# wangheda/youtube-8m

Hardware: AMD Instinct MI355X
Metric: training videos/sec (higher is better)
Workload: dtype f32; 1 GPU; BASELINE configs[3]: LstmModel (2 x BasicLSTMCell(1024), dynamic_rnn over F=300) on raw uint8 [B,300,1152] frames + MoeModel head (2 mixtures, V=4716), fp32 training step (fwd+bwd+clip+Adam); per_gpu_batch=128, global_batch=128, frames=300, parallelism=dp1, params=113902808

## Files before the change

### include/yt8m_hip.h

```cpp
#ifndef YT8M_HIP_H
#define YT8M_HIP_H
#include <stdint.h>

#ifdef __cplusplus
extern "C" {
#endif

typedef void* yt8m_stream_t;

enum yt8m_status { YT8M_OK = 0, YT8M_E_BADARG = -1, YT8M_E_SHAPE = -2, YT8M_E_HIP = -3, YT8M_E_RCCL = -4 };
enum yt8m_label_dtype { YT8M_LABEL_U8 = 0, YT8M_LABEL_F32 = 1 };

int yt8m_abi_version(void);
const char* yt8m_last_error(void);
const char* yt8m_built_arch(void);

int yt8m_prof_enable(int on);
int yt8m_prof_reset(void);
int yt8m_prof_get(int family, int64_t* launches, double* total_ms);
int yt8m_prof_get_flops(int family, double* flops);
int yt8m_prof_get_bytes(int family, double* bytes);

int yt8m_probe_mfma_f32(int iters, int blocks, float* sink, yt8m_stream_t stream);
int yt8m_probe_mfma_bf16(int iters, int blocks, int random_operands, float* sink, yt8m_stream_t stream);
// ... 49 lines not shown
                          yt8m_stream_t stream);
int yt8m_timepool_shiftmax_f32(const float* z, int64_t F, int64_t B, int64_t ldz, int nfilt, const int32_t* fs, const int32_t* ncol, float* out,
                               int32_t* idx, int64_t ldo, yt8m_stream_t stream);
int yt8m_u8_cnn_pool_dw(const uint8_t* q, const float* r_tm, const int32_t* idx, const float* g, int64_t ldg, int64_t B, int64_t F, int64_t D,
                        int64_t N, int64_t fs, float* dW, float beta, yt8m_stream_t stream);
int yt8m_f32_cnn_pool_dw(const float* x, int64_t ldx, const int32_t* idx, const float* g, int64_t ldg, int64_t B, int64_t F, int64_t D,
                         int64_t N, int64_t fs, float* dW, int64_t lddw, float beta, yt8m_stream_t stream);
int yt8m_f32_cnn_pool_dx(const int32_t* idx, const float* g, int64_t ldg, int64_t B, int64_t F, int64_t D, int nfilt, const float* const* wt,
                         const int32_t* fs, const int32_t* ncol, float* dx, int64_t lddx, yt8m_stream_t stream);
int yt8m_u8_frames_image_f16(const uint8_t* q, const int32_t* num_frames, int64_t B, int64_t F, int64_t D, float eps, void* image,
                             float* x_tm, float* r_out, yt8m_stream_t stream);
int yt8m_u8_frames_image_t_f16(const uint8_t* q, const int32_t* num_frames, int64_t B, int64_t F, int64_t D, void* image_t,
                               yt8m_stream_t stream);
int yt8m_gemm_h2_nt_grouped(int nprob, const yt8m_gemm_problem* probs, const float* alphas, const float* const* dsa,
                            const float* const* dsb, void* workspace, int64_t workspace_bytes, yt8m_stream_t stream);
int yt8m_x3_set_combine(int mode);
int yt8m_x3_set_schedule(int mode);
#define YT8M_GEMM_ROLE_DW 0x100
#define YT8M_GEMM_ROLE_H2 0x200
int yt8m_gemm_x3_pays(int64_t M, int64_t N, int64_t K);
int64_t yt8m_gemm_auto_scratch_bytes(int transA, int transB, int nprob, const yt8m_gemm_problem* probs);
int yt8m_gemm_auto_grouped(int transA, int transB, int nprob, const yt8m_gemm_problem* probs, void* workspace,
                           int64_t workspace_bytes, void* image_scratch, int64_t image_scratch_bytes, uint64_t* used_x3,
                           yt8m_stream_t stream);
int yt8m_gemm_auto_grouped_ex(int transA, int transB, int nprob, const yt8m_gemm_problem* probs, const float* const* absmaxA,
                              const float* const* absmaxB, void* workspace, int64_t workspace_bytes, void* image_scratch,
                              int64_t image_scratch_bytes, uint64_t* used_x3, yt8m_stream_t stream);
int yt8m_gemm_x1x3_nt(int64_t M, int64_t N, int64_t K, const void* A1, const void* B3, float* C, int64_t ldc, const float* bias,
                      const float* rowscale, const float* colsum, float colsum_scale, void* workspace, int64_t workspace_bytes,
                      yt8m_stream_t stream);
// ... 332 lines not shown
int64_t yt8m_lstm_stack_tape_bytes(const yt8m_lstm_stack_desc* desc);
int64_t yt8m_lstm_stack_scratch_bytes(const yt8m_lstm_stack_desc* desc);
int yt8m_lstm_stack_partition(const yt8m_lstm_stack_desc* desc, int* fwd_chunks, int* bwd_chunks);
int yt8m_lstm_stack_streams(int L, yt8m_stream_t* layer_streams, yt8m_stream_t* wgrad_stream);
int yt8m_lstm_stack_fwd(const yt8m_lstm_stack_desc* desc, const void* x, const int32_t* num_frames, const float* const* W,
                        const float* const* b, void* tape, int64_t tape_bytes, void* scratch, int64_t scratch_bytes,
                        yt8m_stream_t stream);
int yt8m_lstm_stack_view(const yt8m_lstm_stack_desc* desc, void* tape, int layer, int which, float** out);
int yt8m_lstm_stack_bwd(const yt8m_lstm_stack_desc* desc, const void* x, const int32_t* num_frames, const float* const* W, void* tape,
                        int64_t tape_bytes, void* scratch, int64_t scratch_bytes, const float* dout_top,
                        const float* const* dc_final, const float* const* dh_final, float* const* dW, float* const* db,
                        const float* beta_W, const float* beta_b, float* dx, yt8m_stream_t stream);
int yt8m_lstm_stack_status(const yt8m_lstm_stack_desc* desc, void* scratch, yt8m_stream_t stream);
int yt8m_lstm_stack_layer_done_wait(int layer, yt8m_stream_t stream);
int yt8m_lstm_stack_use_streams(int set, int* previous);
typedef void (*yt8m_stream_hook)(void* user, yt8m_stream_t stream);
int yt8m_lstm_stack_set_prep_hook(yt8m_stream_hook hook, void* user);
typedef struct yt8m_opt_ranges {
  float* w;
  float* m;
  float* v;
  const float* g;
  const int32_t* chunks;
  const int32_t* tensor_chunk_start;
  const int32_t* tensor_chunk_start_host;
  const float* l2;
  float* partial;
  float* norms;
  const uint8_t* skip_tensor;
  const yt8m_wimg_job* jobs;
// ... 217 lines not shown
```

### youtube-8m_amd/_lib.py

```python
import ctypes
import os

_HERE = os.path.dirname(os.path.abspath(__file__))
LIB_PATH = os.environ.get("YT8M_LIB", os.path.join(_HERE, "libyt8m_hip.so"))

c_void_p, c_int, c_int64, c_float, c_double = ctypes.c_void_p, ctypes.c_int, ctypes.c_int64, ctypes.c_float, ctypes.c_double
P = c_void_p

class GemmProblem(ctypes.Structure):
    _fields_ = [("M", c_int64), ("N", c_int64), ("K", c_int64), ("A", c_void_p), ("lda", c_int64), ("B", c_void_p),
                ("ldb", c_int64), ("C", c_void_p), ("ldc", c_int64), ("bias", c_void_p), ("beta", c_float)]


STREAM_HOOK = ctypes.CFUNCTYPE(None, ctypes.c_void_p, ctypes.c_void_p)


class PersistBwdImages(ctypes.Structure):
    _fields_ = [("plain", ctypes.c_void_p), ("trans", ctypes.c_void_p), ("trans_scaled", ctypes.c_void_p), ("rowscale", ctypes.c_void_p),
                ("colpart", ctypes.c_void_p), ("colpart_scaled", ctypes.c_void_p)]


class LstmStackDesc(ctypes.Structure):
    _fields_ = [("B", c_int64), ("F", c_int64), ("D", c_int64), ("H", c_int64), ("L", ctypes.c_int32), ("input_u8", ctypes.c_int32),
                ("forget_bias", c_float), ("fwd_chunks", ctypes.c_int32), ("bwd_chunks", ctypes.c_int32), ("need_dx", ctypes.c_int32),
# ... 283 lines not shown
    "yt8m_gemm_h1x2_nt_ex": (c_int, [c_int64, c_int64, c_int64, P, c_int64, P, c_int64, P, c_int64, P, c_float, P, P, P, c_float, c_float, P,
                                     c_int64, P]),
    "yt8m_h2_rowscales": (c_int, [P, c_int64, c_int64, c_int64, P, P, P]),
    "yt8m_h2_split_rows": (c_int, [P, c_int64, c_int64, c_int64, P, P, P]),
    "yt8m_gemm_h2_nt_ex": (c_int, [c_int64, c_int64, c_int64, P, c_int64, P, c_int64, P, c_int64, P, c_float, P, P, P, c_float, P, c_int64, P]),
    "yt8m_timepool_max_f32": (c_int, [P, c_int64, c_int64, c_int64, c_int64, P, P, c_int64, P]),
    "yt8m_timepool_shiftmax_f32": (c_int, [P, c_int64, c_int64, c_int64, c_int, ctypes.POINTER(ctypes.c_int32), ctypes.POINTER(ctypes.c_int32), P, P,
                                           c_int64, P]),
    "yt8m_u8_cnn_pool_dw": (c_int, [P, P, P, P, c_int64, c_int64, c_int64, c_int64, c_int64, c_int64, P, c_float, P]),
    "yt8m_f32_cnn_pool_dw": (c_int, [P, c_int64, P, P, c_int64, c_int64, c_int64, c_int64, c_int64, c_int64, P, c_int64, c_float, P]),
    "yt8m_f32_cnn_pool_dx": (c_int, [P, P, c_int64, c_int64, c_int64, c_int64, c_int, PP, ctypes.POINTER(ctypes.c_int32),
                                     ctypes.POINTER(ctypes.c_int32), P, c_int64, P]),
    "yt8m_u8_frames_image_f16": (c_int, [P, P, c_int64, c_int64, c_int64, c_float, P, P, P, P]),
    "yt8m_u8_frames_image_t_f16": (c_int, [P, P, c_int64, c_int64, c_int64, P, P]),
    "yt8m_gemm_h2_nt_grouped": (c_int, [c_int, ctypes.POINTER(GemmProblem), ctypes.POINTER(c_float), PP, PP, P, c_int64, P]),
    "yt8m_topk_rows": (c_int, [P, c_int64, c_int64, c_int, P, P, P]),
    "yt8m_perr_rows": (c_int, [P, P, c_int64, c_int64, P, P]),
    "yt8m_reverse_sequence_u8": (c_int, [P, P, P, c_int64, c_int64, c_int64, P]),
    "yt8m_reverse_sequence_f32_tm": (c_int, [P, c_int64, P, P, c_int64, c_int64, c_int64, c_int64, c_int64, P]),
    "yt8m_lstm_stack_use_streams": (c_int, [c_int, ctypes.POINTER(c_int)]),
    "yt8m_half_segments_u8": (c_int, [P, P, P, P, c_int64, c_int64, c_int64, P]),
    "yt8m_half_segments_f32": (c_int, [P, P, P, P, c_int64, c_int64, c_int64, P]),
    "yt8m_half_segment_means_u8": (c_int, [P, P, P, c_int64, c_int64, c_int64, c_int, c_float, P]),
    "yt8m_dequant_noise_u8": (c_int, [P, P, P, c_int64, c_int64, c_int64, c_float, ctypes.c_uint64, P]),
    "yt8m_resolution_mean_u8": (c_int, [P, P, P, P, c_int64, c_int64, c_int64, c_int64, c_int, c_float, P]),
    "yt8m_resolution_mean_f32": (c_int, [P, P, P, P, c_int64, c_int64, c_int64, c_int64, c_int, c_float, P]),
    "yt8m_multiscale_workspace_bytes": (c_int64, [c_int64]),
    "yt8m_colmoments_f32": (c_int, [P, c_int64, c_int64, c_int64, P, P, c_int, c_float, c_float, P, P, P, c_int64, P]),
    "yt8m_bn_relu_pool2_tm_fwd": (c_int, [P, c_int64, c_int64, c_int64, c_int64, P, P, P, P, P, c_int64, P, c_int64, P]),
    "yt8m_bn_relu_pool2_tm_bwd": (c_int, [P, c_int64, c_int64, c_int64, c_int64, P, P, P, P, c_int, P, c_int64, P, c_int64, P, c_int64, P,
# ... 73 lines not shown
```

### youtube-8m_amd/csrc/gemm_x3.hip

```cpp
#include "common.h"
#include "x3_image.h"
#include "philox.h"
#include <type_traits>
#include <algorithm>
#include <mutex>
#include <stdlib.h>

namespace {

constexpr int TM = 256, TN = 256;
constexpr int PLANE_F = 256 * 8;
constexpr int OP_F = 3 * PLANE_F;
constexpr int NST = 3;
using yt8m_x3::RG_F;
using yt8m_x3::store_block;

typedef float f32x16 __attribute__((ext_vector_type(16)));
typedef __bf16 bf16x8 __attribute__((ext_vector_type(8)));

struct XArgs {
  const float* A;
  const float* B;
  float* C;
  const float* bias;
  int64_t ldc;
  int M, N, KB;
  int ska, skb;
  int tiles_m, tiles_n;
  int accumulate;
  const float* rscale;
  const float* cs;
  float cs_scale;
  float alpha;
  const float* dsa;
  const float* dsb;
  int c_bf16;
};
__device__ __forceinline__ unsigned c_bf16_bits(float f) {
  unsigned u = __float_as_uint(f);
  if ((u & 0x7fffffffu) > 0x7f800000u) return (u >> 16) | 0x40u;
  u += 0x7fffu + ((u >> 16) & 1u);
  return u >> 16;
}
__device__ __forceinline__ void store_c4(const XArgs& g, int64_t off, float4 v) {
  if (g.c_bf16) {
    uint2 w;
    w.x = c_bf16_bits(v.x) | (c_bf16_bits(v.y) << 16);
    w.y = c_bf16_bits(v.z) | (c_bf16_bits(v.w) << 16);
    *reinterpret_cast<uint2*>(reinterpret_cast<unsigned short*>(g.C) + off) = w;
  } else {
    *reinterpret_cast<float4*>(g.C + off) = v;
// ... 513 lines not shown
      step(kt + 1, a0y, b2y, a0x, b2x, variant);
    }
    if (kt < nk) step(kt, a0x, b2x, a0y, b2y, variant);
  };
  if (grp == 0) run(std::integral_constant<int, 0>{});
  else run(std::integral_constant<int, 1>{});
  asm volatile("s_waitcnt lgkmcnt(0)" ::: "memory");
  __builtin_amdgcn_s_barrier();

  x_epilogue(G, g, acc, smem, m0, n0, wm, wn, lane, wave, li, lk, nparts, slot, q, lt);
}

typedef _Float16 f16x8 __attribute__((ext_vector_type(8)));

template <int PA>
__global__ __launch_bounds__(512) void gemm_h2q_kernel(const XGroup G) {
  constexpr int OPA_F = PA * PLANE_F;
  constexpr int H2_STAGE_F = (PA + 2) * PLANE_F;
  extern __shared__ __attribute__((aligned(16))) float smem[];
  int q, nparts, part, slot, lt;
  x_work_item(G, q, nparts, part, slot, lt);
  const XArgs& g = G.p[q];
  int tm, tn;
  tile_coords(g.tiles_m, g.tiles_n, lt, tm, tn);
  const int m0 = tm * TM, n0 = tn * TN;
  const int tid = threadIdx.x, lane = tid & 63, wave = tid >> 6;
  const int grp = wave >> 2;
  const int wm = grp * 128, wn = (wave & 3) * 64;
  const int li = lane & 31, lk = lane >> 5;
  const int kb0 = (int)((int64_t)g.KB * part / nparts), kb1 = (int)((int64_t)g.KB * (part + 1) / nparts);
  const int nk = kb1 - kb0;
  const float* pa = g.A + (int64_t)min(m0 / 32 + wave, (g.M + 31) / 32 - 1) * g.ska * (PA * RG_F) + lane * 4;
  const float* pb = g.B + (int64_t)min(n0 / 32 + wave, (g.N + 31) / 32 - 1) * g.skb * (2 * RG_F) + lane * 4;
  constexpr int DMA = PA + 2;
  f32x16 acc[4][2];
#pragma unroll
// ... 99 lines not shown
    int kt = 0;
    for (; kt + 1 < nk; kt += 2) {
      step(kt, ahx, blx, ahy, bly, variant);
      step(kt + 1, ahy, bly, ahx, blx, variant);
    }
    if (kt < nk) step(kt, ahx, blx, ahy, bly, variant);
  };
  if (grp == 0) run(std::integral_constant<int, 0>{});
  else run(std::integral_constant<int, 1>{});
  asm volatile("s_waitcnt lgkmcnt(0)" ::: "memory");
  __builtin_amdgcn_s_barrier();

  const XArgs ge = fold_device_scales(g);
  x_epilogue(G, ge, acc, smem, m0, n0, wm, wn, lane, wave, li, lk, nparts, slot, q, lt);
}

constexpr int B1_KBS = 4;
constexpr int B1_STAGE_F = 2 * B1_KBS * PLANE_F;

__global__ __launch_bounds__(512) void gemm_b1_kernel(const XGroup G) {
  extern __shared__ __attribute__((aligned(16))) float smem[];
  int q, nparts, part, slot, lt;
  x_work_item(G, q, nparts, part, slot, lt);
  const XArgs& g = G.p[q];
  int tm, tn;
  tile_coords(g.tiles_m, g.tiles_n, lt, tm, tn);
  const int m0 = tm * TM, n0 = tn * TN;
  const int tid = threadIdx.x, lane = tid & 63, wave = tid >> 6;
  const int wm = (wave >> 2) * 128, wn = (wave & 3) * 64;
  const int li = lane & 31, lk = lane >> 5;
// ... 627 lines not shown
        return nullptr;
      }
      base[dev] = p;
    }
    if (next[dev] + (uint32_t)n > CNT_CAP) next[dev] = 0;
    unsigned* r = base[dev] + next[dev];
    next[dev] += (uint32_t)n;
    return r;
  }
};
TileCounters g_cnt;

template <int PA>
int x3_launch(int nprob, const yt8m_gemm_problem* probs, const float* rscale, const float* cs, float cs_scale, float alpha,
              void* workspace, int64_t workspace_bytes, yt8m_stream_t stream, const float* const* dsa = nullptr,
              const float* const* dsb = nullptr, const float* alphas = nullptr, unsigned c_bf16_mask = 0) {
  XGroup G;
  G.nprob = 0;
  static const int SLOTS_ENV = getenv("YT8M_X3_SLOTS") ? atoi(getenv("YT8M_X3_SLOTS")) : 0;
  const int SLOTS = SLOTS_ENV >= 32 && SLOTS_ENV <= 256 ? SLOTS_ENV : 256;
  const int64_t per_part = (int64_t)TM * TN * sizeof(float);
  int64_t nfull = 0, slots = 0, fix = 0;
  for (int i = 0; i < nprob; ++i) {
    const yt8m_gemm_problem& q = probs[i];
    YT8M_REQUIRE(q.M >= 0 && q.N >= 0 && q.K >= 1 && q.ldc >= q.N, YT8M_E_BADARG, "bad GEMM problem");
    YT8M_REQUIRE(q.beta == 0.f || q.beta == 1.f, YT8M_E_BADARG, "beta must be 0 or 1");
    if (q.M == 0 || q.N == 0) continue;
    YT8M_REQUIRE(q.A && q.B && q.C, YT8M_E_BADARG, "null operand");
    YT8M_REQUIRE((((uintptr_t)q.A | (uintptr_t)q.B) & 15) == 0, YT8M_E_BADARG, "x3 images must be 16-byte aligned");
    XArgs g;
    g.A = static_cast<const float*>(q.A); g.B = static_cast<const float*>(q.B); g.C = q.C; g.bias = q.bias;
    g.ldc = q.ldc;
    g.M = (int)q.M; g.N = (int)q.N; g.KB = (int)((q.K + 15) / 16);
    YT8M_REQUIRE(q.lda >= 0 && q.ldb >= 0 && q.lda < (1LL << 30) && q.ldb < (1LL << 30) && (q.lda == 0 || q.lda >= g.KB) &&
                 (q.ldb == 0 || q.ldb >= g.KB), YT8M_E_BADARG, "bad image K-block stride");
    YT8M_REQUIRE((q.lda <= g.KB && q.ldb <= g.KB) || (q.K % 16) == 0, YT8M_E_SHAPE, "a K range of a larger image must be a multiple of 16");
    g.ska = q.lda ? (int)q.lda : g.KB; g.skb = q.ldb ? (int)q.ldb : g.KB;
    g.tiles_m = (int)((q.M + TM - 1) / TM); g.tiles_n = (int)((q.N + TN - 1) / TN);
    g.accumulate = q.beta != 0.f;
    g.rscale = rscale; g.cs = cs; g.cs_scale = cs_scale; g.alpha = alphas ? alphas[i] : alpha;
    g.dsa = dsa ? dsa[i] : nullptr; g.dsb = dsb ? dsb[i] : nullptr;
    g.c_bf16 = (int)((c_bf16_mask >> i) & 1u);
    YT8M_REQUIRE(!g.c_bf16 || (q.beta == 0.f && (q.ldc & 3) == 0 && ((uintptr_t)q.C & 15) == 0), YT8M_E_BADARG,
                 "a bf16 output takes beta = 0, ldc % 4 == 0 and a 16-byte aligned C");
    YT8M_REQUIRE(!(g.dsa || g.dsb || g.alpha != 1.0f) || (q.N % 4) == 0, YT8M_E_SHAPE, "a scaled product needs N % 4 == 0");
    const int64_t T = (int64_t)g.tiles_m * g.tiles_n;
    const int full = (int)(T / SLOTS) * SLOTS, rem = (int)(T - full);
    int S = 1;
    if (workspace && rem > 0) {
      double best = 1e30;
      for (int c = 1; c <= 16; ++c) {
        if (c > 1 && (g.KB / c < (PA == 0 ? 32 : 8) || (slots + (int64_t)rem * c) * per_part > workspace_bytes)) break;
        const int rounds = (rem * c + SLOTS - 1) / SLOTS;
        const double cost = rounds * ((double)g.KB / c + 10.0) + (c > 1 ? 4.0 + 0.065 * rem * c : 0.0);
        if (cost < best * 0.98) { best = cost; S = c; }
      }
    }
// ... 6 lines not shown
    G.part_base[k] = (int)slots;
    G.slot_base[k] = (int)slots;
    G.fix_base[k] = (int)fix;
    nfull += G.full[k];
    if (S > 1) { slots += (int64_t)rem * S; fix += rem; }
    ++G.nprob;
  }
  if (G.nprob == 0) return YT8M_OK;
  YT8M_REQUIRE(nfull + slots < (1LL << 30), YT8M_E_SHAPE, "too many tiles for one launch");
  for (int i = G.nprob; i <= 4; ++i) { G.full_base[i] = (int)nfull; G.part_base[i] = (int)slots; G.fix_base[i] = (int)fix; }
  for (int i = G.nprob; i < 4; ++i) { G.p[i] = G.p[0]; G.S[i] = 1; G.slot_base[i] = 0; G.full[i] = 0; G.rem[i] = 0; }
  G.ws = static_cast<float*>(workspace);
  G.cnt = fix > 0 ? g_cnt.take((int)fix) : nullptr;
  const int64_t grid = nfull + slots;
  constexpr int LDS_BYTES = PA == 0 ? 2 * B1_STAGE_F * (int)sizeof(float)
                            : PA == 2 ? NST * 4 * PLANE_F * (int)sizeof(float)
                            : PA == 4 ? NST * 3 * PLANE_F * (int)sizeof(float) : NST * (PA + 3) * PLANE_F * (int)sizeof(float);
  static DeviceOnce lds_once;
  if constexpr (PA == 0) YT8M_HIP_CHECK(lds_once.lds(reinterpret_cast<const void*>(gemm_b1_kernel), LDS_BYTES));
  else if constexpr (PA == 2) YT8M_HIP_CHECK(lds_once.lds(reinterpret_cast<const void*>(gemm_h2q_kernel<2>), LDS_BYTES));
  else if constexpr (PA == 4) YT8M_HIP_CHECK(lds_once.lds(reinterpret_cast<const void*>(gemm_h2q_kernel<1>), LDS_BYTES));
  else YT8M_HIP_CHECK(lds_once.lds(reinterpret_cast<const void*>(gemm_x3_kernel<(PA == 1) ? 1 : 3>), LDS_BYTES));
  double fl = 0.0;
  for (int i = 0; i < nprob; ++i) fl += 2.0 * (double)probs[i].M * (double)probs[i].N * (double)probs[i].K;
  ProfScope prof(PA == 0 ? F_GEMM : (PA == 1 ? F_GEMM_X1X3 : (PA == 2 ? F_GEMM_H2 : (PA == 4 ? F_GEMM_H1X2 : F_GEMM_X3))), as_stream(stream), fl);
  static const bool piped_env = getenv("YT8M_B1_PIPE") == nullptr || atoi(getenv("YT8M_B1_PIPE")) != 0;
  const bool piped = g_schedule_mode == 1 || (g_schedule_mode == 0 && piped_env);
  const char* launched = "gemm_x3_kernel";
  if constexpr (PA == 0) {
    launched = piped ? "gemm_b1q_kernel" : "gemm_b1_kernel";
    if (piped) {
      static DeviceOnce lds_once_q;
      YT8M_HIP_CHECK(lds_once_q.lds(reinterpret_cast<const void*>(gemm_b1q_kernel), BQ_SLOTS * BQ_SLOT_F * (int)sizeof(float)));
      hipLaunchKernelGGL(gemm_b1q_kernel, dim3((unsigned)grid), dim3(512), BQ_SLOTS * BQ_SLOT_F * (int)sizeof(float), as_stream(stream), G);
    } else {
      hipLaunchKernelGGL(gemm_b1_kernel, dim3((unsigned)grid), dim3(512), LDS_BYTES, as_stream(stream), G);
    }
  }
  else if constexpr (PA == 2) {
    launched = "gemm_h2q_kernel";
    hipLaunchKernelGGL(gemm_h2q_kernel<2>, dim3((unsigned)grid), dim3(512), LDS_BYTES, as_stream(stream), G);
  }
  else if constexpr (PA == 4) {
    launched = "gemm_h2q_kernel";
    hipLaunchKernelGGL(gemm_h2q_kernel<1>, dim3((unsigned)grid), dim3(512), LDS_BYTES, as_stream(stream), G);
  }
  else {
    static const bool xpiped_env = getenv("YT8M_X3_PIPE") == nullptr || atoi(getenv("YT8M_X3_PIPE")) != 0;
    const bool xpiped = g_schedule_mode == 1 || (g_schedule_mode == 0 && xpiped_env);
    launched = xpiped ? "gemm_x3q_kernel" : "gemm_x3_kernel";
    if (xpiped) {
      static DeviceOnce lds_once_xq;
      YT8M_HIP_CHECK(lds_once_xq.lds(reinterpret_cast<const void*>(gemm_x3q_kernel<(PA == 1) ? 1 : 3>), LDS_BYTES));
      hipLaunchKernelGGL(gemm_x3q_kernel<(PA == 1) ? 1 : 3>, dim3((unsigned)grid), dim3(512), LDS_BYTES, as_stream(stream), G);
    } else {
      hipLaunchKernelGGL(gemm_x3_kernel<(PA == 1) ? 1 : 3>, dim3((unsigned)grid), dim3(512), LDS_BYTES, as_stream(stream), G);
    }
  }
  if (fix > 0 && !G.cnt) hipLaunchKernelGGL(x3_fixup_kernel, dim3((unsigned)fix * 16), dim3(256), 0, as_stream(stream), G);
  return launch_status(launched);
}
// ... 23 lines not shown
  return x3_launch<0>(nprob, probs, nullptr, nullptr, 0.f, 1.0f, workspace, workspace_bytes, stream);
}

extern "C" int yt8m_gemm_b1_nt_grouped_bf16c(int nprob, const yt8m_gemm_problem* probs, unsigned c_bf16_mask, void* workspace,
                                             int64_t workspace_bytes, yt8m_stream_t stream) {
  YT8M_REQUIRE(nprob >= 1 && nprob <= 4 && probs, YT8M_E_BADARG, "1..4 problems per launch");
  return x3_launch<0>(nprob, probs, nullptr, nullptr, 0.f, 1.0f, workspace, workspace_bytes, stream, nullptr, nullptr, nullptr, c_bf16_mask);
}

extern "C" int yt8m_gemm_h2_nt_grouped(int nprob, const yt8m_gemm_problem* probs, const float* alphas, const float* const* dsa,
                                       const float* const* dsb, void* workspace, int64_t workspace_bytes, yt8m_stream_t stream) {
  YT8M_REQUIRE(nprob >= 1 && nprob <= 4 && probs, YT8M_E_BADARG, "1..4 problems per launch");
  return x3_launch<2>(nprob, probs, nullptr, nullptr, 0.f, 1.0f, workspace, workspace_bytes, stream, dsa, dsb, alphas);
}

extern "C" int yt8m_gemm_h2_nt_ex(int64_t M, int64_t N, int64_t K, const void* A2, int64_t ska, const void* B2, int64_t skb, float* C,
                                  int64_t ldc, const float* bias, float alpha, const void* dsa, const void* dsb, const float* rowscale,
                                  float beta, void* workspace, int64_t workspace_bytes, yt8m_stream_t stream) {
  YT8M_REQUIRE((N % 4) == 0, YT8M_E_SHAPE, "the scaled epilogue needs N % 4 == 0");
  yt8m_gemm_problem p;
  p.M = M; p.N = N; p.K = K; p.A = A2; p.lda = ska; p.B = B2; p.ldb = skb; p.C = C; p.ldc = ldc; p.bias = bias; p.beta = beta;
  const float* wa = static_cast<const float*>(dsa);
  const float* wb = static_cast<const float*>(dsb);
  return x3_launch<2>(1, &p, rowscale, nullptr, 0.f, alpha, workspace, workspace_bytes, stream, dsa ? &wa : nullptr, dsb ? &wb : nullptr);
}

extern "C" int yt8m_gemm_h1x2_nt_ex(int64_t M, int64_t N, int64_t K, const void* A1, int64_t ska, const void* B2, int64_t skb, float* C,
                                    int64_t ldc, const float* bias, float alpha, const void* dsb, const float* rowscale, const float* colsum,
                                    float colsum_scale, float beta, void* workspace, int64_t workspace_bytes, yt8m_stream_t stream) {
  YT8M_REQUIRE((N % 4) == 0, YT8M_E_SHAPE, "the scaled epilogue needs N % 4 == 0");
// ... 38 lines not shown
```

### youtube-8m_amd/csrc/lstm_stack.hip

```cpp
#include <stdlib.h>
#include <algorithm>
#include <mutex>
#include <vector>
#include "common.h"

using namespace yt8m;

namespace {

constexpr int MAXL = 8, MAXP = 64;
constexpr int MAXBP = 62;
constexpr float U8_ALPHA = 4.0f / 255.0f;
constexpr float U8_BETA = 128.0f * (4.0f / 255.0f) + (4.0f / 512.0f - 2.0f);
constexpr int64_t X3_MIN_ROWS = 1024;
constexpr int64_t STEP_IMAGES_MAX_BYTES = 8LL << 30;
constexpr float H2_S = 8192.0f;

int64_t up256(int64_t v) { return (v + 255) / 256 * 256; }

int knob(const char* name, int dflt) { const char* v = getenv(name); return v ? atoi(v) : dflt; }

struct Part { int64_t t0, T; };
int chunks(int64_t F, int n, Part* out) {
  if (n < 1) n = 1;
// ... 111 lines not shown
  int64_t fmax = 0, bmax = 0;
  for (int c = 0; c < p.nf; ++c) fmax = std::max(fmax, p.fp[c].T * p.B);
  for (int c = 0; c < p.nb; ++c) bmax = std::max(bmax, p.bp[c].T * p.B);
  for (int l = 0; l < p.L; ++l) {
    const int64_t Din = l ? p.H : p.D;
    const bool x1 = l == 0 && p.u8;
    p.wxt3[l] = o; o += x1 ? 0 : up256(ib(H4, Din));
    p.xi[l] = o; o += x1 ? 0 : up256(ib(fmax, Din));
    p.dz[l] = o; o += up256(FBH * 4 * 4);
    p.dbuf[l] = o; o += l + 1 < p.L ? up256(FBH * 4) : 0;
    p.work[l] = o; o += up256(4 * BH * 4);
    const bool dxl = l > 0 || p.need_dx;
    p.dz3[l] = o; o += dxl ? up256(ib(bmax, H4)) : 0;
    p.wx3[l] = o; o += dxl ? up256(ib(Din, H4)) : 0;
    p.xT[l] = o; o += x1 ? up256(x1_bytes(p.D, p.FB)) : up256(ib(Din, p.FB));
    p.hT[l] = o; o += up256(ib(p.H, p.FB));
  }
  p.h2 = (knob("YT8M_STACK_H2", 1) && !p.bf16) ? 1 : 0;
  p.keep = (d->input_keep_prob > 0.f && d->input_keep_prob < 1.f) ? d->input_keep_prob : 0.f;
  for (int l = 0; l < MAXL; ++l) p.seed[l] = d->dropout_seed[l];
  if (d->input_keep_prob < 0.f || d->input_keep_prob > 1.f) return "input_keep_prob must be in [0, 1]";
  if (p.keep > 0.f && (p.u8 || !p.h2 || p.keep < 0.3f || (p.D % 4) != 0 || (p.H % 4) != 0))
    return "input dropout: float input, f16 product forms (YT8M_STACK_H2), keep_prob >= 0.3, D % 4 == 0";
  p.img_rows = (knob("YT8M_STACK_FUSED_IMAGES", 0) && !p.bf16 && !p.h2) ? yt8m_lstm_persist_bwd_images_rows(p.B, p.H) : 0;
  const int64_t trows = p.img_rows ? p.FB : bmax;
  for (int l = 0; l < p.L; ++l) { p.dzT3[l] = o; o += up256(ib(H4, trows)); }
  p.dzT3s = o; o += p.u8 ? up256(ib(H4, trows)) : 0;
  const int64_t ci = p.img_rows ? up256((int64_t)p.img_rows * MAXP * 2 * H4 * 4) : 0;
  for (int l = 0; l < p.L; ++l) { p.cimg[l] = o; o += ci; }
  p.cimgs = o; o += p.u8 ? ci : 0;
  p.csr = o; o += up256(H4 * 4);
// ... 121 lines not shown

extern "C" int yt8m_lstm_stack_streams(int L, yt8m_stream_t* layer_streams, yt8m_stream_t* wgrad_stream) {
  YT8M_REQUIRE(L >= 1 && L <= MAXL && layer_streams, YT8M_E_BADARG, "1..8 layers, non-null output");
  std::lock_guard<std::mutex> lk(g_mu);
  DevState* S = nullptr;
  RC(dev_state(L, &S));
  for (int l = 0; l < L; ++l) layer_streams[l] = (yt8m_stream_t)S->rs[l];
  if (wgrad_stream) *wgrad_stream = (yt8m_stream_t)S->sw;
  return YT8M_OK;
}

extern "C" int yt8m_lstm_stack_use_streams(int set, int* previous) {
  YT8M_REQUIRE(set >= 0 && set < NSETS, YT8M_E_BADARG, "stream set must be 0 or 1");
  if (previous) *previous = g_set;
  g_set = set;
  return YT8M_OK;
}

extern "C" int yt8m_lstm_stack_view(const yt8m_lstm_stack_desc* desc, void* tape, int layer, int which, float** out) {
  Plan P;
  const char* why = plan(desc, &P);
  YT8M_REQUIRE(!why, YT8M_E_SHAPE, why ? why : "");
  YT8M_REQUIRE(tape && out && layer >= 0 && layer < P.L && which >= 0 && which <= 3, YT8M_E_BADARG, "bad view");
  const int64_t FBH = P.FB * P.H;
  switch (which) {
    case 0: *out = at<float>(tape, P.out[layer]); break;
    case 1: *out = at<float>(tape, P.cs[layer]) + FBH; break;
    case 2: *out = at<float>(tape, P.hs[layer]) + FBH; break;
    default: *out = at<float>(tape, P.z[layer]); break;
  }
// ... 218 lines not shown
  YT8M_REQUIRE(!P.need_dx || dx, YT8M_E_BADARG, "need_dx is set but dx is NULL");
  for (int l = 0; l < P.L; ++l) {
    YT8M_REQUIRE(W[l], YT8M_E_BADARG, "null weights");
    YT8M_REQUIRE(!beta_W || beta_W[l] == 0.f || beta_W[l] == 1.f, YT8M_E_BADARG, "beta must be 0 or 1");
    YT8M_REQUIRE(!beta_b || beta_b[l] == 0.f || beta_b[l] == 1.f, YT8M_E_BADARG, "beta must be 0 or 1");
  }
  std::lock_guard<std::mutex> lk(g_mu);
  DevState* S = nullptr;
  RC(dev_state(P.L, &S));
  Ev ev(*S, 1);
  hipStream_t main = as_stream(stream), sw = S->sw;
  static const int dx_stream = knob("YT8M_STACK_DX_STREAM", 0), two_sw = knob("YT8M_STACK_SW2", 0);
  const int fuse_dz = P.h2 ? 0 : knob("YT8M_STACK_FUSE_DZ_SPLIT", 0);
  const int64_t B = P.B, D = P.D, H = P.H, H4 = 4 * H, BH = B * H, FB = P.FB;
  const int64_t KBtot = FB / 16;
  const bool bf = P.bf16 != 0;
  const int64_t KBB = bf ? 1024 : 3072;
  auto split = [&](const float* src, int64_t R, int64_t C, int64_t ld, float scale, void* plain, void* trans, hipStream_t st) {
    return bf ? yt8m_bf16_image(src, R, C, ld, scale, plain, trans, (yt8m_stream_t)st) : yt8m_x3_split(src, R, C, ld, scale, plain, trans, (yt8m_stream_t)st);
  };
  auto gemm = [&](int n, const yt8m_gemm_problem* pr, void* ws, int64_t wsb, hipStream_t st) {
    return bf ? yt8m_gemm_b1_nt_grouped(n, pr, ws, wsb, (yt8m_stream_t)st) : yt8m_gemm_x3_nt_grouped(n, pr, ws, wsb, (yt8m_stream_t)st);
  };
  hipEvent_t start = ev.record(main);
  ev.wait(sw, start);
  if (two_sw) ev.wait(S->sw2, start);
  for (int l = 0; l < P.L; ++l) { ev.wait(S->rs[l], start); if (dx_stream) ev.wait(S->dxs[l], start); }
  if (P.h2)
    for (int l = 0; l < P.L; ++l) {
      YT8M_HIP_CHECK(hipMemsetAsync(at<char>(scratch, P.hsc + 256 * l + 4), 0, 248, S->rs[l]));
      if (P.emit_max && l >= 1) YT8M_HIP_CHECK(hipMemsetAsync(at<char>(scratch, P.rmax + l * P.rmax_stride), 0, (size_t)FB * 4, S->rs[l]));
    }
  for (int l = 0; l < P.L; ++l) {
    if (!dW[l]) continue;
    if (l == 0 && P.u8) {
      if (P.h2) RC(yt8m_u8_frames_image_t_f16(static_cast<const uint8_t*>(x), num_frames, B, P.F, D, at<char>(scratch, P.xT[0]), sw));
      else RC(yt8m_u8_frames_image_t(static_cast<const uint8_t*>(x), num_frames, B, P.F, D, at<char>(scratch, P.xT[0]), sw));
    } else {
      const float* src = l ? at<float>(tape, P.out[l - 1]) : static_cast<const float*>(x);
      const int64_t Din = l ? H : D;
      if (P.h2 && P.keep > 0.f)
        RC(yt8m_h2_split_dropout(src, FB, Din, l ? H2_S : 1.0f, l ? nullptr : at<float>(scratch, P.hx0), nullptr, at<char>(scratch, P.xT[l]),
                                 P.keep, P.seed[l], 0, (yt8m_stream_t)sw));
      else if (P.h2 && l >= 1) RC(yt8m_h2_split(src, FB, Din, Din, H2_S, nullptr, nullptr, at<char>(scratch, P.xT[l]), nullptr, (yt8m_stream_t)sw));
      else if (P.h2) RC(yt8m_h2_split(src, FB, Din, Din, 1.0f, at<float>(scratch, P.hx0), nullptr, at<char>(scratch, P.xT[0]), nullptr, (yt8m_stream_t)sw));
      else RC(split(src, FB, Din, Din, 1.0f, nullptr, at<char>(scratch, P.xT[l]), sw));
    }
    if (P.h2) RC(yt8m_h2_split(at<float>(tape, P.hs[l]), FB, H, H, H2_S, nullptr, nullptr, at<char>(scratch, P.hT[l]), nullptr, (yt8m_stream_t)sw));
    else RC(split(at<float>(tape, P.hs[l]), FB, H, H, 1.0f, nullptr, at<char>(scratch, P.hT[l]), sw));
  }
  yt8m_stream_hook hook = g_prep_hook;
  void* hook_user = g_prep_user;
  g_prep_hook = nullptr;
  g_prep_user = nullptr;
  bool early = g_early.set;
  g_early.set = false;
  if (two_sw) ev.wait(S->sw2, ev.record(sw));
  int phase[MAXL];
  bool wx3_done[MAXL];
  const void* wx_img[MAXL] = {nullptr};
  hipEvent_t dzT_free[MAXL] = {nullptr};
  const bool fused_img = P.img_rows > 0 && !dx_stream && !fuse_dz;
  int64_t img_done_rows[MAXL] = {0};
// ... 145 lines not shown
      }
      hipStream_t sw = (two_sw && l == 0) ? S->sw2 : S->sw;
      ev.wait(sw, rb);
      void* gw = at<char>(scratch, (two_sw && l == 0) ? P.gws2 : P.gws[P.L]);
      const float bW = first ? (beta_W ? beta_W[l] : 0.f) : 1.f;
      const bool lastpart = c == 0 && j == 0;
      if (dW[l]) {
        if (l == 0 && P.u8 && P.h2) {
          const float* rr = at<float>(tape, P.rrow) + t0 * B;
          float* word = at<float>(scratch, P.hsc) + 1 + c;
          if (!P.emit_max) RC(yt8m_h2_absmax(dzc, M, H4, H4, word, (yt8m_stream_t)sw));
          float* cp = P.colparts ? at<float>(scratch, P.cpart[l]) + (t0 * B / 64) * H4 : nullptr;
          float* cps = P.colparts ? at<float>(scratch, P.cparts) + (t0 * B / 64) * H4 : nullptr;
          RC(yt8m_h2_split_ex(dzc, M, H4, H4, 1.0f, word, rr, nullptr, at<char>(scratch, P.dzT3[l]), at<char>(scratch, P.dzT3s), cp, cps,
                              (yt8m_stream_t)sw));
          RC(yt8m_gemm_h1x2_nt_ex(D, H4, M, at<char>(scratch, P.xT[0]) + kb0 * 1024, KBtot, at<char>(scratch, P.dzT3s), 0, dW[0], H4, nullptr,
                                  U8_ALPHA, word, nullptr, nullptr, 0.f, bW, gw, P.gws_bytes, (yt8m_stream_t)sw));
          yt8m_gemm_problem pr = {H, H4, M, at<char>(scratch, P.hT[0]) + kb0 * 2048, KBtot, at<char>(scratch, P.dzT3[l]), 0,
                                  dW[0] + D * H4, H4, nullptr, bW};
          const float alpha = 1.0f / H2_S;
          const float* dsb = word;
          RC(yt8m_gemm_h2_nt_grouped(1, &pr, &alpha, nullptr, &dsb, gw, P.gws_bytes, (yt8m_stream_t)sw));
        } else if (l == 0 && P.u8) {
          const float* rr = at<float>(tape, P.rrow) + t0 * B;
          if (fused_img) {
          } else if (P.colparts || bf) {
            float* cp = P.colparts ? at<float>(scratch, P.cpart[l]) + (t0 * B / 64) * H4 : nullptr;
            float* cps = P.colparts ? at<float>(scratch, P.cparts) + (t0 * B / 64) * H4 : nullptr;
            if (bf) RC(yt8m_bf16_image_colsum(dzc, M, H4, H4, 1.0f, rr, nullptr, at<char>(scratch, P.dzT3[l]), at<char>(scratch, P.dzT3s), cp, cps, sw));
            else RC(yt8m_x3_split_colsum(dzc, M, H4, H4, 1.0f, rr, nullptr, at<char>(scratch, P.dzT3[l]), at<char>(scratch, P.dzT3s), cp, cps, sw));
          } else
            RC(yt8m_x3_split_ex(dzc, M, H4, H4, 1.0f, rr, nullptr, at<char>(scratch, P.dzT3[l]), at<char>(scratch, P.dzT3s), sw));
          if (bf)
            RC(yt8m_gemm_b1_nt_ex(D, H4, M, at<char>(scratch, P.xT[0]) + kb0 * 1024, KBtot, dzTs_img, 0, dW[0], H4,
                                  nullptr, U8_ALPHA, nullptr, nullptr, 0.f, bW, gw, P.gws_bytes, sw));
          else
            RC(yt8m_gemm_x1x3_nt_ex(D, H4, M, at<char>(scratch, P.xT[0]) + kb0 * 1024, KBtot, dzTs_img, 0, dW[0], H4,
                                    nullptr, U8_ALPHA, nullptr, nullptr, 0.f, bW, gw, P.gws_bytes, sw));
          yt8m_gemm_problem pr = {H, H4, M, at<char>(scratch, P.hT[0]) + kb0 * KBB, KBtot, dzT_img, 0,
                                  dW[0] + D * H4, H4, nullptr, bW};
          RC(gemm(1, &pr, gw, P.gws_bytes, sw));
        } else if (P.h2) {
          float* word = at<float>(scratch, P.hsc + 256 * l) + 1 + c;
          if (!P.emit_max) RC(yt8m_h2_absmax(dzc, M, H4, H4, word, (yt8m_stream_t)sw));
          float* cp = (P.colparts && db[l]) ? at<float>(scratch, P.cpart[l]) + (t0 * B / 64) * H4 : nullptr;
          RC(yt8m_h2_split(dzc, M, H4, H4, 1.0f, word, nullptr, at<char>(scratch, P.dzT3[l]), cp, (yt8m_stream_t)sw));
          yt8m_gemm_problem pr[2] = {
              {Din, H4, M, at<char>(scratch, P.xT[l]) + kb0 * 2048, KBtot, at<char>(scratch, P.dzT3[l]), 0, dW[l], H4, nullptr, bW},
              {H, H4, M, at<char>(scratch, P.hT[l]) + kb0 * 2048, KBtot, at<char>(scratch, P.dzT3[l]), 0, dW[l] + Din * H4, H4, nullptr, bW}};
          const float alphas[2] = {l ? 1.0f / H2_S : 1.0f, 1.0f / H2_S};
          const float* dsa[2] = {l ? nullptr : at<float>(scratch, P.hx0), nullptr};
          const float* dsb[2] = {word, word};
          RC(yt8m_gemm_h2_nt_grouped(2, pr, alphas, dsa, dsb, gw, P.gws_bytes, (yt8m_stream_t)sw));
        } else {
          if (fused_img) {
          } else if (!fused_t) {
            if (P.colparts && db[l]) {
              float* cp = at<float>(scratch, P.cpart[l]) + (t0 * B / 64) * H4;
              if (bf) RC(yt8m_bf16_image_colsum(dzc, M, H4, H4, 1.0f, nullptr, nullptr, at<char>(scratch, P.dzT3[l]), nullptr, cp, nullptr, sw));
              else RC(yt8m_x3_split_colsum(dzc, M, H4, H4, 1.0f, nullptr, nullptr, at<char>(scratch, P.dzT3[l]), nullptr, cp, nullptr, sw));
            } else {
              RC(split(dzc, M, H4, H4, 1.0f, nullptr, at<char>(scratch, P.dzT3[l]), sw));
            }
          }
// ... 42 lines not shown
```

Before: 8408 videos/s.

## Group layer-0 u8 dW GEMMs into one mixed-plane launch and share h-transpose images

Adds a mixed-plane grouped h2 GEMM kernel that dispatches per problem between 1-plane and 2-plane A operands, so the layer-0 input-weight and recurrent-weight gradient GEMMs run in one launch instead of two. It also widens the hidden-state transposed image by B rows, so layer l's input image can reuse layer l-1's hT image offset by one timestep and its separate h2 split is skipped. This saves a kernel launch and a split pass per chunk. In exchange it adds a runtime branch in the kernel, which may raise register pressure for the templated instantiation, and uses slightly larger scratch.

New measurement: 8477 videos/s, median of 6. Within noise of the previous version (+0.8%).

```diff
diff --git a/include/yt8m_hip.h b/include/yt8m_hip.h
--- a/include/yt8m_hip.h
+++ b/include/yt8m_hip.h
@@ -87,6 +87,9 @@
                                yt8m_stream_t stream);
 int yt8m_gemm_h2_nt_grouped(int nprob, const yt8m_gemm_problem* probs, const float* alphas, const float* const* dsa,
                             const float* const* dsb, void* workspace, int64_t workspace_bytes, yt8m_stream_t stream);
+int yt8m_gemm_h2_nt_grouped_planes(int nprob, const yt8m_gemm_problem* probs, const int* a_planes, const float* alphas,
+                                   const float* const* dsa, const float* const* dsb, void* workspace, int64_t workspace_bytes,
+                                   yt8m_stream_t stream);
 int yt8m_x3_set_combine(int mode);
 int yt8m_x3_set_schedule(int mode);
 #define YT8M_GEMM_ROLE_DW 0x100
@@ -449,6 +452,7 @@
 int yt8m_lstm_stack_status(const yt8m_lstm_stack_desc* desc, void* scratch, yt8m_stream_t stream);
 int yt8m_lstm_stack_layer_done_wait(int layer, yt8m_stream_t stream);
 int yt8m_lstm_stack_use_streams(int set, int* previous);
+int yt8m_lstm_stack_set_dw_group(int mode);
 typedef void (*yt8m_stream_hook)(void* user, yt8m_stream_t stream);
 int yt8m_lstm_stack_set_prep_hook(yt8m_stream_hook hook, void* user);
 typedef struct yt8m_opt_ranges {
diff --git a/youtube-8m_amd/_lib.py b/youtube-8m_amd/_lib.py
--- a/youtube-8m_amd/_lib.py
+++ b/youtube-8m_amd/_lib.py
@@ -321,6 +321,9 @@
     "yt8m_u8_frames_image_f16": (c_int, [P, P, c_int64, c_int64, c_int64, c_float, P, P, P, P]),
     "yt8m_u8_frames_image_t_f16": (c_int, [P, P, c_int64, c_int64, c_int64, P, P]),
     "yt8m_gemm_h2_nt_grouped": (c_int, [c_int, ctypes.POINTER(GemmProblem), ctypes.POINTER(c_float), PP, PP, P, c_int64, P]),
+    "yt8m_gemm_h2_nt_grouped_planes": (c_int, [c_int, ctypes.POINTER(GemmProblem), ctypes.POINTER(c_int), ctypes.POINTER(c_float), PP, PP, P,
+                                               c_int64, P]),
+    "yt8m_lstm_stack_set_dw_group": (c_int, [c_int]),
     "yt8m_topk_rows": (c_int, [P, c_int64, c_int64, c_int, P, P, P]),
     "yt8m_perr_rows": (c_int, [P, P, c_int64, c_int64, P, P]),
     "yt8m_reverse_sequence_u8": (c_int, [P, P, P, c_int64, c_int64, c_int64, P]),
diff --git a/youtube-8m_amd/csrc/gemm_x3.hip b/youtube-8m_amd/csrc/gemm_x3.hip
--- a/youtube-8m_amd/csrc/gemm_x3.hip
+++ b/youtube-8m_amd/csrc/gemm_x3.hip
@@ -4,6 +4,7 @@
 #include <type_traits>
 #include <algorithm>
 #include <mutex>
+#include <optional>
 #include <stdlib.h>
 
 namespace {
@@ -35,6 +36,7 @@
   const float* dsa;
   const float* dsb;
   int c_bf16;
+  int a_planes;
 };
 __device__ __forceinline__ unsigned c_bf16_bits(float f) {
   unsigned u = __float_as_uint(f);
@@ -578,12 +580,10 @@
 typedef _Float16 f16x8 __attribute__((ext_vector_type(8)));
 
 template <int PA>
-__global__ __launch_bounds__(512) void gemm_h2q_kernel(const XGroup G) {
+__device__ __forceinline__ void h2q_work_item(const XGroup& G, int q, int nparts, int part, int slot, int lt) {
   constexpr int OPA_F = PA * PLANE_F;
   constexpr int H2_STAGE_F = (PA + 2) * PLANE_F;
   extern __shared__ __attribute__((aligned(16))) float smem[];
-  int q, nparts, part, slot, lt;
-  x_work_item(G, q, nparts, part, slot, lt);
   const XArgs& g = G.p[q];
   int tm, tn;
   tile_coords(g.tiles_m, g.tiles_n, lt, tm, tn);
@@ -713,6 +713,17 @@
   const XArgs ge = fold_device_scales(g);
   x_epilogue(G, ge, acc, smem, m0, n0, wm, wn, lane, wave, li, lk, nparts, slot, q, lt);
 }
+template <int PA>
+__global__ __launch_bounds__(512) void gemm_h2q_kernel(const XGroup G) {
+  int q, nparts, part, slot, lt;
+  x_work_item(G, q, nparts, part, slot, lt);
+  if constexpr (PA == 0) {
+    if (G.p[q].a_planes == 1) h2q_work_item<1>(G, q, nparts, part, slot, lt);
+    else h2q_work_item<2>(G, q, nparts, part, slot, lt);
+  } else {
+    h2q_work_item<PA>(G, q, nparts, part, slot, lt);
+  }
+}
 
 constexpr int B1_KBS = 4;
 constexpr int B1_STAGE_F = 2 * B1_KBS * PLANE_F;
@@ -1370,7 +1381,7 @@
 template <int PA>
 int x3_launch(int nprob, const yt8m_gemm_problem* probs, const float* rscale, const float* cs, float cs_scale, float alpha,
               void* workspace, int64_t workspace_bytes, yt8m_stream_t stream, const float* const* dsa = nullptr,
-              const float* const* dsb = nullptr, const float* alphas = nullptr, unsigned c_bf16_mask = 0) {
+              const float* const* dsb = nullptr, const float* alphas = nullptr, unsigned c_bf16_mask = 0, const int* a_planes = nullptr) {
   XGroup G;
   G.nprob = 0;
   static const int SLOTS_ENV = getenv("YT8M_X3_SLOTS") ? atoi(getenv("YT8M_X3_SLOTS")) : 0;
@@ -1397,6 +1408,7 @@
     g.rscale = rscale; g.cs = cs; g.cs_scale = cs_scale; g.alpha = alphas ? alphas[i] : alpha;
     g.dsa = dsa ? dsa[i] : nullptr; g.dsb = dsb ? dsb[i] : nullptr;
     g.c_bf16 = (int)((c_bf16_mask >> i) & 1u);
+    g.a_planes = PA == 6 ? a_planes[i] : 0;
     YT8M_REQUIRE(!g.c_bf16 || (q.beta == 0.f && (q.ldc & 3) == 0 && ((uintptr_t)q.C & 15) == 0), YT8M_E_BADARG,
                  "a bf16 output takes beta = 0, ldc % 4 == 0 and a 16-byte aligned C");
     YT8M_REQUIRE(!(g.dsa || g.dsb || g.alpha != 1.0f) || (q.N % 4) == 0, YT8M_E_SHAPE, "a scaled product needs N % 4 == 0");
@@ -1433,16 +1445,21 @@
   G.cnt = fix > 0 ? g_cnt.take((int)fix) : nullptr;
   const int64_t grid = nfull + slots;
   constexpr int LDS_BYTES = PA == 0 ? 2 * B1_STAGE_F * (int)sizeof(float)
-                            : PA == 2 ? NST * 4 * PLANE_F * (int)sizeof(float)
+                            : (PA == 2 || PA == 6) ? NST * 4 * PLANE_F * (int)sizeof(float)
                             : PA == 4 ? NST * 3 * PLANE_F * (int)sizeof(float) : NST * (PA + 3) * PLANE_F * (int)sizeof(float);
   static DeviceOnce lds_once;
   if constexpr (PA == 0) YT8M_HIP_CHECK(lds_once.lds(reinterpret_cast<const void*>(gemm_b1_kernel), LDS_BYTES));
   else if constexpr (PA == 2) YT8M_HIP_CHECK(lds_once.lds(reinterpret_cast<const void*>(gemm_h2q_kernel<2>), LDS_BYTES));
   else if constexpr (PA == 4) YT8M_HIP_CHECK(lds_once.lds(reinterpret_cast<const void*>(gemm_h2q_kernel<1>), LDS_BYTES));
+  else if constexpr (PA == 6) YT8M_HIP_CHECK(lds_once.lds(reinterpret_cast<const void*>(gemm_h2q_kernel<0>), LDS_BYTES));
   else YT8M_HIP_CHECK(lds_once.lds(reinterpret_cast<const void*>(gemm_x3_kernel<(PA == 1) ? 1 : 3>), LDS_BYTES));
-  double fl = 0.0;
-  for (int i = 0; i < nprob; ++i) fl += 2.0 * (double)probs[i].M * (double)probs[i].N * (double)probs[i].K;
-  ProfScope prof(PA == 0 ? F_GEMM : (PA == 1 ? F_GEMM_X1X3 : (PA == 2 ? F_GEMM_H2 : (PA == 4 ? F_GEMM_H1X2 : F_GEMM_X3))), as_stream(stream), fl);
+  double fl = 0.0, fl1 = 0.0;
+  for (int i = 0; i < nprob; ++i)
+    (PA == 6 && a_planes[i] == 1 ? fl1 : fl) += 2.0 * (double)probs[i].M * (double)probs[i].N * (double)probs[i].K;
+  ProfScope prof(PA == 0 ? F_GEMM : (PA == 1 ? F_GEMM_X1X3 : ((PA == 2 || PA == 6) ? F_GEMM_H2 : (PA == 4 ? F_GEMM_H1X2 : F_GEMM_X3))),
+                 as_stream(stream), fl);
+  std::optional<ProfScope> prof1;
+  if constexpr (PA == 6) prof1.emplace(F_GEMM_H1X2, as_stream(stream), fl1);
   static const bool piped_env = getenv("YT8M_B1_PIPE") == nullptr || atoi(getenv("YT8M_B1_PIPE")) != 0;
   const bool piped = g_schedule_mode == 1 || (g_schedule_mode == 0 && piped_env);
   const char* launched = "gemm_x3_kernel";
@@ -1464,6 +1481,10 @@
     launched = "gemm_h2q_kernel";
     hipLaunchKernelGGL(gemm_h2q_kernel<1>, dim3((unsigned)grid), dim3(512), LDS_BYTES, as_stream(stream), G);
   }
+  else if constexpr (PA == 6) {
+    launched = "gemm_h2q_kernel";
+    hipLaunchKernelGGL(gemm_h2q_kernel<0>, dim3((unsigned)grid), dim3(512), LDS_BYTES, as_stream(stream), G);
+  }
   else {
     static const bool xpiped_env = getenv("YT8M_X3_PIPE") == nullptr || atoi(getenv("YT8M_X3_PIPE")) != 0;
     const bool xpiped = g_schedule_mode == 1 || (g_schedule_mode == 0 && xpiped_env);
@@ -1517,6 +1538,21 @@
   return x3_launch<2>(nprob, probs, nullptr, nullptr, 0.f, 1.0f, workspace, workspace_bytes, stream, dsa, dsb, alphas);
 }
 
+extern "C" int yt8m_gemm_h2_nt_grouped_planes(int nprob, const yt8m_gemm_problem* probs, const int* a_planes, const float* alphas,
+                                              const float* const* dsa, const float* const* dsb, void* workspace, int64_t workspace_bytes,
+                                              yt8m_stream_t stream) {
+  YT8M_REQUIRE(nprob >= 1 && nprob <= 4 && probs && a_planes, YT8M_E_BADARG, "1..4 problems per launch, each with its plane count");
+  int ones = 0;
+  for (int i = 0; i < nprob; ++i) {
+    YT8M_REQUIRE(a_planes[i] == 1 || a_planes[i] == 2, YT8M_E_BADARG, "a_planes must be 1 or 2");
+    YT8M_REQUIRE(a_planes[i] == 2 || !dsa || !dsa[i], YT8M_E_BADARG, "a one-plane A operand is exact: no scale word");
+    ones += a_planes[i] == 1;
+  }
+  if (ones == 0) return x3_launch<2>(nprob, probs, nullptr, nullptr, 0.f, 1.0f, workspace, workspace_bytes, stream, dsa, dsb, alphas);
+  if (ones == nprob) return x3_launch<4>(nprob, probs, nullptr, nullptr, 0.f, 1.0f, workspace, workspace_bytes, stream, nullptr, dsb, alphas);
+  return x3_launch<6>(nprob, probs, nullptr, nullptr, 0.f, 1.0f, workspace, workspace_bytes, stream, dsa, dsb, alphas, 0, a_planes);
+}
+
 extern "C" int yt8m_gemm_h2_nt_ex(int64_t M, int64_t N, int64_t K, const void* A2, int64_t ska, const void* B2, int64_t skb, float* C,
                                   int64_t ldc, const float* bias, float alpha, const void* dsa, const void* dsb, const float* rowscale,
                                   float beta, void* workspace, int64_t workspace_bytes, yt8m_stream_t stream) {
diff --git a/youtube-8m_amd/csrc/lstm_stack.hip b/youtube-8m_amd/csrc/lstm_stack.hip
--- a/youtube-8m_amd/csrc/lstm_stack.hip
+++ b/youtube-8m_amd/csrc/lstm_stack.hip
@@ -149,7 +149,7 @@
     p.dz3[l] = o; o += dxl ? up256(ib(bmax, H4)) : 0;
     p.wx3[l] = o; o += dxl ? up256(ib(Din, H4)) : 0;
     p.xT[l] = o; o += x1 ? up256(x1_bytes(p.D, p.FB)) : up256(ib(Din, p.FB));
-    p.hT[l] = o; o += up256(ib(p.H, p.FB));
+    p.hT[l] = o; o += up256(ib(p.H, p.FB + p.B));
   }
   p.h2 = (knob("YT8M_STACK_H2", 1) && !p.bf16) ? 1 : 0;
   p.keep = (d->input_keep_prob > 0.f && d->input_keep_prob < 1.f) ? d->input_keep_prob : 0.f;
@@ -301,6 +301,13 @@
   YT8M_REQUIRE(set >= 0 && set < NSETS, YT8M_E_BADARG, "stream set must be 0 or 1");
   if (previous) *previous = g_set;
   g_set = set;
+  return YT8M_OK;
+}
+
+static thread_local int g_dw_group = 0;
+extern "C" int yt8m_lstm_stack_set_dw_group(int mode) {
+  YT8M_REQUIRE(mode >= 0 && mode <= 2, YT8M_E_BADARG, "mode must be 0 (default), 1 (grouped) or 2 (separate launches)");
+  g_dw_group = mode;
   return YT8M_OK;
 }
 
@@ -549,6 +556,11 @@
   const int fuse_dz = P.h2 ? 0 : knob("YT8M_STACK_FUSE_DZ_SPLIT", 0);
   const int64_t B = P.B, D = P.D, H = P.H, H4 = 4 * H, BH = B * H, FB = P.FB;
   const int64_t KBtot = FB / 16;
+  const bool grouped = g_dw_group != 2;
+  const bool share_h = grouped && P.h2 && P.keep == 0.f && B % 16 == 0;
+  const int64_t KBh = share_h ? KBtot + B / 16 : KBtot;
+  const int64_t hrows = share_h ? FB + B : FB;
+  auto x_shared = [&](int l) { return share_h && l >= 1 && dW[l - 1] != nullptr; };
   const bool bf = P.bf16 != 0;
   const int64_t KBB = bf ? 1024 : 3072;
   auto split = [&](const float* src, int64_t R, int64_t C, int64_t ld, float scale, void* plain, void* trans, hipStream_t st) {
@@ -577,11 +589,12 @@
       if (P.h2 && P.keep > 0.f)
         RC(yt8m_h2_split_dropout(src, FB, Din, l ? H2_S : 1.0f, l ? nullptr : at<float>(scratch, P.hx0), nullptr, at<char>(scratch, P.xT[l]),
                                  P.keep, P.seed[l], 0, (yt8m_stream_t)sw));
+      else if (x_shared(l)) {}
       else if (P.h2 && l >= 1) RC(yt8m_h2_split(src, FB, Din, Din, H2_S, nullptr, nullptr, at<char>(scratch, P.xT[l]), nullptr, (yt8m_stream_t)sw));
       else if (P.h2) RC(yt8m_h2_split(src, FB, Din, Din, 1.0f, at<float>(scratch, P.hx0), nullptr, at<char>(scratch, P.xT[0]), nullptr, (yt8m_stream_t)sw));
       else RC(split(src, FB, Din, Din, 1.0f, nullptr, at<char>(scratch, P.xT[l]), sw));
     }
-    if (P.h2) RC(yt8m_h2_split(at<float>(tape, P.hs[l]), FB, H, H, H2_S, nullptr, nullptr, at<char>(scratch, P.hT[l]), nullptr, (yt8m_stream_t)sw));
+    if (P.h2) RC(yt8m_h2_split(at<float>(tape, P.hs[l]), hrows, H, H, H2_S, nullptr, nullptr, at<char>(scratch, P.hT[l]), nullptr, (yt8m_stream_t)sw));
     else RC(split(at<float>(tape, P.hs[l]), FB, H, H, 1.0f, nullptr, at<char>(scratch, P.hT[l]), sw));
   }
   yt8m_stream_hook hook = g_prep_hook;
@@ -757,13 +770,19 @@
           float* cps = P.colparts ? at<float>(scratch, P.cparts) + (t0 * B / 64) * H4 : nullptr;
           RC(yt8m_h2_split_ex(dzc, M, H4, H4, 1.0f, word, rr, nullptr, at<char>(scratch, P.dzT3[l]), at<char>(scratch, P.dzT3s), cp, cps,
                               (yt8m_stream_t)sw));
-          RC(yt8m_gemm_h1x2_nt_ex(D, H4, M, at<char>(scratch, P.xT[0]) + kb0 * 1024, KBtot, at<char>(scratch, P.dzT3s), 0, dW[0], H4, nullptr,
-                                  U8_ALPHA, word, nullptr, nullptr, 0.f, bW, gw, P.gws_bytes, (yt8m_stream_t)sw));
-          yt8m_gemm_problem pr = {H, H4, M, at<char>(scratch, P.hT[0]) + kb0 * 2048, KBtot, at<char>(scratch, P.dzT3[l]), 0,
-                                  dW[0] + D * H4, H4, nullptr, bW};
-          const float alpha = 1.0f / H2_S;
-          const float* dsb = word;
-          RC(yt8m_gemm_h2_nt_grouped(1, &pr, &alpha, nullptr, &dsb, gw, P.gws_bytes, (yt8m_stream_t)sw));
+          yt8m_gemm_problem pr[2] = {
+              {D, H4, M, at<char>(scratch, P.xT[0]) + kb0 * 1024, KBtot, at<char>(scratch, P.dzT3s), 0, dW[0], H4, nullptr, bW},
+              {H, H4, M, at<char>(scratch, P.hT[0]) + kb0 * 2048, KBh, at<char>(scratch, P.dzT3[l]), 0, dW[0] + D * H4, H4, nullptr, bW}};
+          const float alphas[2] = {U8_ALPHA, 1.0f / H2_S};
+          const float* dsb[2] = {word, word};
+          if (grouped) {
+            const int planes[2] = {1, 2};
+            RC(yt8m_gemm_h2_nt_grouped_planes(2, pr, planes, alphas, nullptr, dsb, gw, P.gws_bytes, (yt8m_stream_t)sw));
+          } else {
+            RC(yt8m_gemm_h1x2_nt_ex(D, H4, M, pr[0].A, KBtot, pr[0].B, 0, dW[0], H4, nullptr, U8_ALPHA, word, nullptr, nullptr, 0.f, bW, gw,
+                                    P.gws_bytes, (yt8m_stream_t)sw));
+            RC(yt8m_gemm_h2_nt_grouped(1, &pr[1], &alphas[1], nullptr, &dsb[1], gw, P.gws_bytes, (yt8m_stream_t)sw));
+          }
         } else if (l == 0 && P.u8) {
           const float* rr = at<float>(tape, P.rrow) + t0 * B;
           if (fused_img) {
@@ -788,9 +807,11 @@
           if (!P.emit_max) RC(yt8m_h2_absmax(dzc, M, H4, H4, word, (yt8m_stream_t)sw));
           float* cp = (P.colparts && db[l]) ? at<float>(scratch, P.cpart[l]) + (t0 * B / 64) * H4 : nullptr;
           RC(yt8m_h2_split(dzc, M, H4, H4, 1.0f, word, nullptr, at<char>(scratch, P.dzT3[l]), cp, (yt8m_stream_t)sw));
+          const bool xs = x_shared(l);
+          const char* xTl = xs ? at<char>(scratch, P.hT[l - 1]) + (kb0 + B / 16) * 2048 : at<char>(scratch, P.xT[l]) + kb0 * 2048;
           yt8m_gemm_problem pr[2] = {
-              {Din, H4, M, at<char>(scratch, P.xT[l]) + kb0 * 2048, KBtot, at<char>(scratch, P.dzT3[l]), 0, dW[l], H4, nullptr, bW},
-              {H, H4, M, at<char>(scratch, P.hT[l]) + kb0 * 2048, KBtot, at<char>(scratch, P.dzT3[l]), 0, dW[l] + Din * H4, H4, nullptr, bW}};
+              {Din, H4, M, xTl, xs ? KBh : KBtot, at<char>(scratch, P.dzT3[l]), 0, dW[l], H4, nullptr, bW},
+              {H, H4, M, at<char>(scratch, P.hT[l]) + kb0 * 2048, KBh, at<char>(scratch, P.dzT3[l]), 0, dW[l] + Din * H4, H4, nullptr, bW}};
           const float alphas[2] = {l ? 1.0f / H2_S : 1.0f, 1.0f / H2_S};
           const float* dsa[2] = {l ? nullptr : at<float>(scratch, P.hx0), nullptr};
           const float* dsb[2] = {word, word};
```
